# yassram/iterative-closest-point

Measured on AMD Instinct MI355X. Metric: ICP iterations/sec (synthetic 1048576-point pair, C4, exact NN), higher is better.
Workload: dtype f64 (30 exact fp64 grid searches (fp32 screen, candidates decided in fp64: the first from cell seeds, the seeded ones the fused grid iteration nn_grid_iter2_kernel, 75% of its queries kept their correspondence by the exclusion certificate without a walk); fp64 transform and reductions)

## Files before the change

### iterative-closest-point_amd/csrc/icp_grid.hip

```cpp
#include <hip/hip_runtime.h>

#include <algorithm>
#include <cmath>
#include <cstdlib>
#include <string>
#include <type_traits>

#include "icp_canon.h"
#include "icp_device.h"
#include "icp_gridbox.h"
#include "icp_kernels.h"

namespace icp {
namespace {

__device__ __forceinline__ double d64g(double px, double py, double pz, double mx, double my,
                                       double mz)
{
    const double dx = px - mx;
    const double dy = py - my;
    const double dz = pz - mz;
    return (dx * dx + dy * dy) + dz * dz;
}

// ... 951 lines not shown
                            const float rem = rc2 - dy * dy - dz * dz;
                            if (rem < 0.0f) {
                                x1 = x0 - 1;
                            } else {
                                const float xw = sqrtf(rem) * (1.0f + 0x1.0p-20f) + xroom;
                                x0 = max(x0, c0[0] + (int)floorf(fmaxf(tr[0] - xw, -1.0f)));
                                x1 = min(x1, c0[0] + (int)floorf(fminf(tr[0] + xw, xspan)));
                            }
#endif
                            if (x0 <= x1) {
                                a0 = gv.start[row + x0];
                                a1 = gv.start[row + x1 + 1];
                            }
                        }
                        k0[v] = a0;
                        pre[v + 1] = pre[v] + (a1 - a0);
                    }
                    if constexpr (kBal) {
                        int K[2 * KR], P[2 * KR + 1];
                        P[0] = 0;
#pragma unroll
                        for (int v = 0; v < KR; ++v) {
                            const int len = pre[v + 1] - pre[v];
                            const int ok0 = __builtin_amdgcn_update_dpp(0, k0[v], 0xB1, 0xf, 0xf, true);
                            const int ol = __builtin_amdgcn_update_dpp(0, len, 0xB1, 0xf, 0xf, true);
                            K[2 * v] = sub ? ok0 : k0[v];
                            K[2 * v + 1] = sub ? k0[v] : ok0;
                            P[2 * v + 1] = P[2 * v] + (sub ? ol : len);
                            P[2 * v + 2] = P[2 * v + 1] + (sub ? len : ol);
                        }
                        const int T = P[2 * KR];
                        for (int f0 = 0; f0 < T; f0 += G * KU) {
                            int kk[KU];
#pragma unroll
                            for (int v = 0; v < KU; ++v) {
                                const int f = f0 + sub + G * v;
                                int pp = K[0] + f;
#pragma unroll
                                for (int w = 1; w < 2 * KR; ++w)
                                    if (f >= P[w]) pp = K[w] + (f - P[w]);
                                kk[v] = f < T ? pp : -1;
                            }
                            float4 mm[KU];
#pragma unroll
                            for (int v = 0; v < KU; ++v) mm[v] = gv.pts32[kk[v] >= 0 ? kk[v] : 0];
#pragma unroll
                            for (int v = 0; v < KU; ++v)
                                if (kk[v] >= 0) test(mm[v], kk[v]);
                        }
                        continue;
                    }
                    const int tot = pre[KR];
                    for (int f0 = 0; f0 < tot; f0 += KU) {
                        int kk[KU];
#pragma unroll
                        for (int v = 0; v < KU; ++v) {
                            const int f = f0 + v;
                            int pp = k0[0] + f;
#pragma unroll
                            for (int w = 1; w < KR; ++w)
                                if (f >= pre[w]) pp = k0[w] + (f - pre[w]);
                            kk[v] = f < tot ? pp : -1;
                        }
                        float4 mm[KU];
#pragma unroll
                        for (int v = 0; v < KU; ++v) mm[v] = gv.pts32[kk[v] >= 0 ? kk[v] : 0];
#pragma unroll
                        for (int v = 0; v < KU; ++v)
                            if (kk[v] >= 0) test(mm[v], kk[v]);
                    }
                }
            }
            if (nc) flush();
        }
        lap(7);
#pragma unroll
        for (int o = 1; o < G; o <<= 1) {
            const double ob = __shfl_xor(best, o, 64);
            const int oi = __shfl_xor(bi, o, 64), ok2 = __shfl_xor(bk, o, 64), ows = __shfl_xor(wset, o, 64);
            const double ox = __shfl_xor(wx, o, 64), oy = __shfl_xor(wy, o, 64), oz = __shfl_xor(wz, o, 64);
            if (ob < best || (ob == best && (unsigned)oi < (unsigned)bi)) {
                best = ob;
                bi = oi;
                bk = ok2;
                wx = ox;
                wy = oy;
                wz = oz;
                wset = ows;
            } else if (ob == best && oi == bi) {
                bk = max(bk, ok2);
                if (!wset && ows) {
                    wx = ox;
                    wy = oy;
                    wz = oz;
                    wset = 1;
                }
            }
        }
        unsigned long long bigm = __ballot(active && !ok && sub == 0);
        nbig += __popcll(bigm);
        if (kIterDbg && dbg) dcnt[3] += __popcll(bigm);
        while (bigm) {
            const int bl = __ffsll((long long)bigm) - 1;
            bigm &= bigm - 1;
            const double bq[3] = {__shfl(q[0], bl, 64), __shfl(q[1], bl, 64), __shfl(q[2], bl, 64)};
            const double be = __shfl(e, bl, 64);
            const int bh = __shfl(h, bl, 64);
            double b2 = INFINITY;
            int bj = -1;
            int d0[3], d1[3];
            if (bh >= 0 && be == be && be < INFINITY && complete_box(bq, be, gv, budget, d0, d1)) {
                b2 = be;
                bj = bh;
                scan_box<64>(bq, d0, d1, gv, lane, b2, bj);
            } else {
                for (int k = lane; k < nm; k += 64) {
                    const double4 m = m4[k];
                    lex_min(b2, bj, d64g(bq[0], bq[1], bq[2], m.x, m.y, m.z), k);
                }
            }
            group_lex_min<64>(b2, bj);
            if (lane / G == bl / G) {
                best = b2;
                bi = bj < 0 ? 0 : bj;
                bk = -1;
                wset = 0;
            }
        }
        lap(8);
        if (active) {
            if (!(ok && bi == h)) {
                if (wset) {
                    y[0] = wx;
                    y[1] = wy;
                    y[2] = wz;
                } else {
                    const double4 w = m4[bi];
                    y[0] = w.x;
                    y[1] = w.y;
                    y[2] = w.z;
                }
            }
            if (sub == 0) {
                idx[t] = bi;
                yx[t] = y[0];
                yy[t] = y[1];
                yz[t] = y[2];
            }
        }
        const IterState *sh_ = fresh();
        const double cp[3] = {sh_->shift_p[0], sh_->shift_p[1], sh_->shift_p[2]};
        const double cy[3] = {sh_->shift_y[0], sh_->shift_y[1], sh_->shift_y[2]};
        const double d[6] = {active ? q[0] - cp[0] : 0.0, active ? q[1] - cp[1] : 0.0, active ? q[2] - cp[2] : 0.0,
                             active ? y[0] - cy[0] : 0.0, active ? y[1] - cy[1] : 0.0, active ? y[2] - cy[2] : 0.0};
        if constexpr (G == 2 && ICP_ITER_LDS_TREE) {
            double *const lf = s_leaf[wave];
#pragma unroll
            for (int k = 0; k < kCanonCols; ++k) {
                double leaf;
                if (k < 6) leaf = 0.0 + d[k];
                else if (k < 15) leaf = 0.0 + d[(k - 6) / 3] * d[3 + (k - 6) % 3];
                else if (k == 15) leaf = 0.0 + ((d[3] * d[3] + d[4] * d[4]) + d[5] * d[5]);
                else if (k == 16) leaf = 0.0 + ((d[0] * d[0] + d[1] * d[1]) + d[2] * d[2]);
                else leaf = active ? 0.0 + e : 0.0;
                if (!active) leaf = 0.0;
                if (sub == 0) lf[k * kLeafStride + u] = leaf;
            }
            __builtin_amdgcn_fence(__ATOMIC_RELEASE, "wavefront");
            __builtin_amdgcn_wave_barrier();
            __builtin_amdgcn_fence(__ATOMIC_ACQUIRE, "wavefront");
            if (lane < kCanonCols) {
                const double *col = lf + lane * kLeafStride;
                double part[4];
#pragma unroll
                for (int g8 = 0; g8 < 4; ++g8) {
                    double v[8];
#pragma unroll
                    for (int j = 0; j < 8; ++j) v[j] = col[8 * g8 + j];
                    part[g8] = ((v[0] + v[1]) + (v[2] + v[3])) + ((v[4] + v[5]) + (v[6] + v[7]));
                }
                acc = acc + ((part[0] + part[1]) + (part[2] + part[3]));
            }
            __builtin_amdgcn_fence(__ATOMIC_RELEASE, "wavefront");
            __builtin_amdgcn_wave_barrier();
            __builtin_amdgcn_fence(__ATOMIC_ACQUIRE, "wavefront");
        } else
#pragma unroll
        for (int k = 0; k < kCanonCols; ++k) {
            double leaf;
            if (k < 6) leaf = 0.0 + d[k];
            else if (k < 15) leaf = 0.0 + d[(k - 6) / 3] * d[3 + (k - 6) % 3];
            else if (k == 15) leaf = 0.0 + ((d[3] * d[3] + d[4] * d[4]) + d[5] * d[5]);
            else if (k == 16) leaf = 0.0 + ((d[0] * d[0] + d[1] * d[1]) + d[2] * d[2]);
            else leaf = active ? 0.0 + e : 0.0;
            if (!active) leaf = 0.0;
            if constexpr (G == 2) {
                const double v = lane_value(wave_tree_odd(leaf), 63);
                if (lane == k) acc = acc + v;
            } else {
                const double v = lane_value(wave_tree_quad(leaf), 63);
                if (lane == k) acc = v;
            }
        }
        lap(9);
    }
    if (kIterDbg && dbg)
        for (int o = 32; o >= 1; o >>= 1) dcnt[4] += __shfl_xor(dcnt[4], o, 64);
    if (kIterDbg && dbg && lane == 0)
        for (int f = 0; f < 12; ++f)
            if (dcnt[f]) atomicAdd(dbg + f, dcnt[f]);
    __shared__ double sh[NW][kCanonCols];
    if (lane < kCanonCols) sh[wave][lane] = acc;
    __syncthreads();
    if (threadIdx.x < kCanonCols) {
        const int k = threadIdx.x;
        double v[4];
#pragma unroll
        for (int j = 0; j < 4; ++j)
            v[j] = H == 1 ? sh[j][k] : 0.0 + (sh[H * j][k] + sh[H * j + H - 1][k]);
        rows[(size_t)k * R + wr] = (v[0] + v[1]) + (v[2] + v[3]);
    }
    __shared__ int s_cnt[2][NW];
    for (int o = 32; o >= 1; o >>= 1) far += __shfl_xor(far, o, 64);
    if (lane == 0) {
        s_cnt[0][wave] = far;
        s_cnt[1][wave] = nbig;
    }
    __syncthreads();
    if (threadIdx.x < 2) {
        int tot = 0;
        for (int w = 0; w < NW; ++w) tot += s_cnt[threadIdx.x][w];
        int *dst = threadIdx.x == 0 ? far_acc : big_count;
        if (tot && dst) atomicAdd(dst, tot);
    }
}

constexpr int kNoBound = (int)0xbf800000u;
constexpr int kIter2Slot = 8;
constexpr int kIter2Tile = kCanonCols * kLeafStride;
static_assert(32 * kIter2Slot + 32 / 2 <= kIter2Tile, "the hand-off slots and the walker list alias the tiles");

#ifndef ICP_ITER2_DBG
#define ICP_ITER2_DBG 0
#endif
#ifndef ICP_ITER2_F64
#define ICP_ITER2_F64 0
#endif
#ifndef ICP_ITER2_KU
#define ICP_ITER2_KU 4
#endif
#ifndef ICP_ITER2_KR
#define ICP_ITER2_KR 3
#endif
#ifndef ICP_ITER2_KCAND
#define ICP_ITER2_KCAND ICP_ITER_KCAND
#endif
#ifndef ICP_ITER2_WAVES
#define ICP_ITER2_WAVES 4
#endif
#ifndef ICP_ITER2_GFLOOR
#define ICP_ITER2_GFLOOR 1
#endif
#ifndef ICP_ITER2_NWG_DEFAULT
#define ICP_ITER2_NWG_DEFAULT 1
#endif
struct Iter2Args {
    int n;
    double *px, *py, *pz, *yx, *yy, *yz;
    int *idx;
    const IterState *st;
    float4 *p32;
    GridView gv;
    int box, budget, nm;
    const double4 *m4;
    double *rows;
    int *far_acc;
    double far_d2;
    int *big_count;
    int xform, xcd_l;
    CertArgs ca;
    unsigned long long *dbg;
};
static_assert(std::is_trivially_copyable<Iter2Args>::value, "passed by value in the kernel-argument segment");
#define ICP_CONST_AS __attribute__((address_space(4)))
__device__ __forceinline__ const Iter2Args &iter2_args()
{
    auto *p = (const ICP_CONST_AS Iter2Args *)__builtin_amdgcn_kernarg_segment_ptr();
    asm volatile("" : "+s"(p));
    return *(const Iter2Args *)p;
}
__device__ __forceinline__ const IterState &iter2_state(const IterState *st)
{
    auto *p = (const ICP_CONST_AS IterState *)st;
    asm volatile("" : "+s"(p));
    return *(const IterState *)p;
}

template <bool A32, class T> __device__ __forceinline__ T &at32(T *b, int i)
{
    if constexpr (A32) return *(T *)((char *)b + (unsigned)i * (unsigned)sizeof(T));
    else return b[i];
}

template <int KR, int KU, int CH, int NWG, bool A32>
__global__ __launch_bounds__(64 * NWG) __attribute__((amdgpu_waves_per_eu(ICP_ITER2_WAVES))) void nn_grid_iter2_kernel(
    Iter2Args args_)
{
    static_assert(CH == 1 || CH == 2, "one or two chunks a task");
    constexpr bool kDbg = ICP_ITER2_DBG != 0;
    unsigned long long dcnt[4] = {0, 0, 0, 0};
    static_assert(NWG == 4 || NWG == 1, "a row or a strand a workgroup");
    constexpr int NW = NWG, QL = 2 / CH;
    __shared__ double s_tile[NW][CH * kIter2Tile];
    const Iter2Args &T = iter2_args();
    const IterState *const st = T.st;
    const unsigned long long dbg_t0 = kDbg ? __builtin_amdgcn_s_memrealtime() : 0ull;
    const int *const ord = NWG == 1 ? T.ca.order : nullptr;
    auto *oaddr = ord ? (const ICP_CONST_AS int *)ord + blockIdx.x : (const ICP_CONST_AS int *)&st->done;
    auto *daddr = (const ICP_CONST_AS int *)&st->done;
    int s_ord, done;
    asm volatile("s_load_dword %0, %2, 0x0\n\ts_load_dword %1, %3, 0x0\n\ts_waitcnt lgkmcnt(0)"
                 : "=&s"(done), "=&s"(s_ord)
                 : "s"(daddr), "s"(oaddr)
                 : "memory");
    if (done) return;
    const int n = T.n, xcd_l = T.xcd_l, xform = T.xform;
    const int lane = threadIdx.x & 63, wave = threadIdx.x >> 6, u = lane / QL, sub = lane % QL;
    const int C = canon_chunks((size_t)n), S = canon_strands((size_t)n), R = canon_rows((size_t)n);
    const int s = NWG == 4 ? xcd_row((int)blockIdx.x, R, xcd_l) * 4 + wave
                : ord ? ((unsigned)s_ord < (unsigned)S ? s_ord : S)
                      : xcd_row((int)blockIdx.x, S, xcd_l > 0 ? 4 * xcd_l : xcd_l);
    const int wr = s >> 2;
    double *const tile = s_tile[wave];
    double *const slots = tile;
    int *const wl = (int *)(tile + 32 * CH * kIter2Slot);
    auto at = [](auto *b, int i) -> auto & { return at32<A32>(b, i); };
    const bool cert_on = T.ca.state != nullptr, cert_in = cert_on && T.ca.valid != 0, two = T.ca.two != 0;
    auto wave_sync = [] {
        __builtin_amdgcn_fence(__ATOMIC_RELEASE, "wavefront");
        __builtin_amdgcn_wave_barrier();
        __builtin_amdgcn_fence(__ATOMIC_ACQUIRE, "wavefront");
    };
    double acc = 0.0;
    int far = 0, nbig = 0, ncert = 0, nwalk = 0;
    auto slot_t = [&](int c, int uu) { return (c + (uu >> 5) * S) * kCanonChunk + (uu & 31); };
    for (int c = s; s < S && c < C; c += CH * S) {
        const int t = slot_t(c, u);
        const bool active = c + (u >> 5) * S < C && t < n;
        if (kDbg) dcnt[0] += 1;
        const Iter2Args &A = iter2_args();
        const Xform xf = iter2_state(st).xf;
        double *const px = A.px, *const py = A.py, *const pz = A.pz, *const yx = A.yx, *const yy = A.yy, *const yz = A.yz;
        int *const idx = A.idx;
        int4 *const cstate = A.ca.state;
        float4 *const p32 = A.p32;
        const double far_d2 = A.far_d2;
        double q[3] = {0.0, 0.0, 0.0}, y[3] = {0.0, 0.0, 0.0};
        int h = -1;
        int4 cs4 = make_int4(kNoBound, kNoBound, -1, -1);
        double mot = 0.0;
        if (active) {
            const double p0 = at(px, t), p1 = at(py, t), p2 = at(pz, t);
            y[0] = at(yx, t);
            y[1] = at(yy, t);
            y[2] = at(yz, t);
            h = at(idx, t);
            if (cert_in) cs4 = at(cstate, t);
            if (xform) {
                transform_point(xf, p0, p1, p2, q[0], q[1], q[2]);
                if (cert_in)
                    mot = (double)(__builtin_amdgcn_sqrtf(__double2float_ru(residual2(p0, p1, p2, q[0], q[1], q[2]))) *
                                   (1.0f + 0x1.0p-21f));
            } else {
                q[0] = p0;
                q[1] = p1;
                q[2] = p2;
            }
        }
        const double e = active ? residual2(y[0], y[1], y[2], q[0], q[1], q[2]) : 0.0;
        if (active && sub == 0 && xform) {
            at(px, t) = q[0];
            at(py, t) = q[1];
            at(pz, t) = q[2];
            if (p32)
                at(p32, t) = make_float4((float)(q[0] - xf.c[0]), (float)(q[1] - xf.c[1]), (float)(q[2] - xf.c[2]),
                                     0.0f);
        }
        if (active && sub == 0) {
            if (far_d2 >= 0.0) {
                if (xform) far += e > far_d2 ? 1 : 0;
            } else if (!(h >= 0 && e * (A.gv.inv_h * A.gv.inv_h) < 2.2)) {
                int b0[3], b1[3];
                far += h >= 0 && e == e && e < INFINITY && complete_box(q, e, A.gv, A.box, b0, b1) ? 0 : 1;
            }
        }
        double best = e;
        int bi = h;
        double w[3] = {y[0], y[1], y[2]};
        bool certd = false;
        const float R1 = __int_as_float(cs4.x), R3 = __int_as_float(cs4.y);
        if (cert_in && active && h >= 0 && (R1 > 0.0f || R3 > 0.0f)) {
            const double R1c = ((double)R1 - mot) - (double)R1 * 0x1.0p-48;
            const double R3c = ((double)R3 - mot) - (double)R3 * 0x1.0p-48;
            auto inside = [](double d2, double r) { return r > 0.0 && d2 * (1.0 + 0x1.0p-38) < r * r * (1.0 - 0x1.0p-50); };
            double R1n = R1c;
            int2 pn = make_int2(cs4.z, cs4.w);
            certd = inside(e, R1c);
            if (kDbg && !certd && two && cs4.w >= 0 && R3c > 0.0) dcnt[3] += 1;
            if (!certd && two && cs4.w >= 0 && R3c > 0.0) {
                const double4 r2 = at(A.gv.pts, cs4.w);
                const double d2 = d64g(q[0], q[1], q[2], r2.x, r2.y, r2.z);
                const int mi2 = (int)r2.w;
                const bool swap = d2 < e || (d2 == e && (unsigned)mi2 < (unsigned)h);
                const double db = swap ? d2 : e;
                if (inside(db, R3c)) {
                    certd = true;
                    const double lb = fmin(R3c, (double)__builtin_amdgcn_sqrtf(__double2float_rd(swap ? e : d2)) * (1.0 - 0x1.0p-21));
                    if (swap) {
                        best = d2;
                        bi = mi2;
                        w[0] = r2.x;
                        w[1] = r2.y;
                        w[2] = r2.z;
                        R1n = lb;
                        pn = make_int2(cs4.w, cs4.z);
                    } else {
                        R1n = fmax(R1c, lb);
                    }
                }
            }
            if (certd && sub == 0) {
                const int4 ns = make_int4(__float_as_int(R1n > 0.0 ? __double2float_rd(R1n) : -1.0f),
                                          __float_as_int(R3c > 0.0 ? __double2float_rd(R3c) : -1.0f), pn.x, pn.y);
                if (bi != h) {
                    at(cstate, t) = ns;
                    at(idx, t) = bi;
                    at(yx, t) = w[0];
                    at(yy, t) = w[1];
                    at(yz, t) = w[2];
                } else {
                    *(int2 *)&at(cstate, t) = make_int2(ns.x, ns.y);
                }
            }
        }
        double *const sl = slots + u * kIter2Slot;
        const bool walker = active && !certd;
        if (walker && sub == 0) {
            sl[0] = q[0];
            sl[1] = q[1];
            sl[2] = q[2];
            sl[3] = best;
            ((int *)(sl + 7))[0] = bi;
            ((int *)(sl + 7))[1] = h;
        }
        if (active && sub == 0) {
            sl[4] = w[0];
            sl[5] = w[1];
            sl[6] = w[2];
        }
        const unsigned long long wm = __ballot(walker && sub == 0);
        ncert += certd && sub == 0 ? 1 : 0;
        nwalk += walker && sub == 0 ? 1 : 0;
        const int nW = __popcll(wm);
        if (walker && sub == 0) wl[__popcll(wm & ((1ull << lane) - 1ull))] = u;
        wave_sync();
        if (kDbg) dcnt[1] += nW;
        for (int b0 = 0; b0 < nW; b0 += 32) {
            const Iter2Args &D = iter2_args();
            const GridView gv = D.gv;
            const int box = D.box;
            const double skin = D.ca.skin;
            if (kDbg) dcnt[2] += 1;
            const int nb = min(32, nW - b0);
            const int lg = nb > 16 ? 1 : nb > 8 ? 2 : nb > 4 ? 3 : nb > 2 ? 4 : nb > 1 ? 5 : 6;
            const int G = ICP_ITER2_GFLOOR ? 64 / nb : 1 << lg;
            const int ginv = (65536 + G - 1) / G;
            const int wi = (lane * ginv) >> 16, ws = lane - wi * G, gbase = wi * G;
            const bool wact = wi < nb;
            const int wu = wl[b0 + (wact ? wi : 0)];
            const double *const ws_sl = slots + wu * kIter2Slot;
            double wq[3], wb = INFINITY;
            int wbi = -1;
            wq[0] = ws_sl[0];
            wq[1] = ws_sl[1];
            wq[2] = ws_sl[2];
            if (wact) {
                wb = ws_sl[3];
                wbi = ((const int *)(ws_sl + 7))[0];
            }
            int c0[3] = {0, 0, 0}, c1[3] = {-1, -1, -1};
            double rw = 0.0, rb = 0.0, s0 = 0.0;
            bool ok = false;
            if (wact && wbi >= 0 && wb == wb && wb < INFINITY) {
                s0 = sqrt(wb);
                if (cert_on) {
                    rw = s0 + skin;
                    rb = rw * (1.0 + 0x1.0p-51);
                    ok = complete_box_r(wq, rb, gv, box, c0, c1);
                }
                if (!ok) {
                    rw = rb = s0;
                    ok = complete_box_r(wq, rb, gv, box, c0, c1);
                }
            }
            if (wact && ws == 0) slots[wu * kIter2Slot + 3] = rw;
            int bk = -1;
            float a1 = INFINITY, a2 = INFINITY;
            int k1 = -1;
            auto other = [&](float v, int k) {
                const bool lt = v < a1;
                a2 = __builtin_amdgcn_fmed3f(a1, v, a2);
                a1 = lt ? v : a1;
                k1 = lt ? k : k1;
            };
            auto eq_of = [&]() {
                const double o0 = wq[0] - gv.c32[0], o1 = wq[1] - gv.c32[1], o2 = wq[2] - gv.c32[2];
                return std::ldexp(fmax(fabs(o0), fmax(fabs(o1), fabs(o2))), -23) + gv.em32;
            };
            double eq = 0.0;
            if (ok) {
                const float f0 = (float)(wq[0] - gv.c32[0]), f1 = (float)(wq[1] - gv.c32[1]), f2 = (float)(wq[2] - gv.c32[2]);
                eq = eq_of();
                const float T = seeded_bound32_root(s0, eq);
                const int ny = c1[1] - c0[1] + 1, nrq = ny * (c1[2] - c0[2] + 1);
                constexpr int kCand = ICP_ITER2_KCAND;
                int cand[kCand], nc = 0;
                auto flush = [&]() {
                    double4 r[kCand];
#pragma unroll
                    for (int j = 0; j < kCand; ++j)
                        if (j < nc) r[j] = at(gv.pts, cand[j]);
#pragma unroll
                    for (int j = 0; j < kCand; ++j) {
                        if (j >= nc) break;
                        const int mi = (int)r[j].w;
                        const double d = d64g(wq[0], wq[1], wq[2], r[j].x, r[j].y, r[j].z);
                        if (d < wb || (d == wb && (unsigned)mi < (unsigned)wbi)) {
                            if (cert_on && bk >= 0) other(__double2float_rd(wb), bk);
                            wb = d;
                            wbi = mi;
                            bk = cand[j];
                        } else if (cert_on) {
                            other(__double2float_rd(d), cand[j]);
                        }
                    }
                    nc = 0;
                };
                auto test = [&](const float4 (&m)[KU], const int (&kk)[KU]) {
                    bool cnd[KU];
                    bool anyc = false;
#pragma unroll
                    for (int v = 0; v < KU; ++v) {
                        const float dx = f0 - m[v].x, dy = f1 - m[v].y, dz = f2 - m[v].z;
                        const float d32 = (dx * dx + dy * dy) + dz * dz;
                        const bool val = kk[v] >= 0, fr = d32 > T;
                        if (cert_on) other(val && fr ? d32 : INFINITY, kk[v]);
                        const bool self = val && !fr && __float_as_int(m[v].w) == wbi;
                        bk = self ? kk[v] : bk;
                        cnd[v] = val && !fr && !self;
                        anyc = anyc || cnd[v];
                    }
                    if (__ballot(anyc)) {
#pragma unroll
                        for (int v = 0; v < KU; ++v)
                            if (cnd[v]) {
                                cand[nc++] = kk[v];
                                if (nc == kCand) flush();
                            }
                    }
                };
                const float inv_ny = 1.0f / (float)ny;
                float tr[3];
#pragma unroll
                for (int a = 0; a < 3; ++a) tr[a] = (float)((wq[a] - gv.lo[a]) * gv.inv_h - (double)c0[a]);
                const float rcf = (float)(rb * gv.inv_h * (1.0 + 0x1.0p-18) +
                                          0x1.0p-20 * (1.0 + fabs((double)tr[0]) + fabs((double)tr[1]) + fabs((double)tr[2])));
                const float rc2 = rcf * rcf, xroom = 0x1.0p-20f * (1.0f + fabsf(tr[0]));
                const float xspan = (float)(c1[0] - c0[0] + 1);
                auto row_run = [&](int r, int &a0, int &a1r) {
                    a0 = 0;
                    a1r = 0;
                    if (r >= nrq) return;
                    const int rz = (int)(((float)r + 0.5f) * inv_ny), ry = r - rz * ny;
                    const int row = ((c0[2] + rz) * gv.g[1] + c0[1] + ry) * gv.g[0];
                    int x0 = c0[0], x1 = c1[0];
                    const float dy = fmaxf(0.0f, fmaxf((float)ry - tr[1], tr[1] - (float)(ry + 1)));
                    const float dz = fmaxf(0.0f, fmaxf((float)rz - tr[2], tr[2] - (float)(rz + 1)));
                    const float rem = rc2 - dy * dy - dz * dz;
                    if (rem < 0.0f) return;
                    const float xw = __builtin_amdgcn_sqrtf(rem) * (1.0f + 0x1.0p-20f) + xroom;
                    x0 = max(x0, c0[0] + (int)floorf(fmaxf(tr[0] - xw, -1.0f)));
                    x1 = min(x1, c0[0] + (int)floorf(fminf(tr[0] + xw, xspan)));
                    if (x0 <= x1) {
                        a0 = at(gv.start, row + x0);
                        a1r = at(gv.start, row + x1 + 1);
                    }
                };
                {
                    for (int r0 = ws; r0 < nrq; r0 += KR * G) {
                        int k0[KR], pre[KR + 1];
                        pre[0] = 0;
#pragma unroll
                        for (int v = 0; v < KR; ++v) {
                            int a0, a1r;
                            row_run(r0 + v * G, a0, a1r);
                            k0[v] = a0;
                            pre[v + 1] = pre[v] + (a1r - a0);
                        }
                        const int tot = pre[KR];
                        for (int f0 = 0; f0 < tot; f0 += KU) {
                            int kk[KU];
#pragma unroll
                            for (int v = 0; v < KU; ++v) {
                                const int f = f0 + v;
                                int pp = k0[0] + f;
#pragma unroll
                                for (int x = 1; x < KR; ++x)
                                    if (f >= pre[x]) pp = k0[x] + (f - pre[x]);
                                kk[v] = f < tot ? pp : -1;
                            }
                            if constexpr (ICP_ITER2_F64) {
                                double4 mm[KU];
#pragma unroll
                                for (int v = 0; v < KU; ++v) mm[v] = at(gv.pts, kk[v] >= 0 ? kk[v] : 0);
#pragma unroll
                                for (int v = 0; v < KU; ++v) {
                                    const double d = d64g(wq[0], wq[1], wq[2], mm[v].x, mm[v].y, mm[v].z);
                                    const int mi = (int)mm[v].w, kv = kk[v];
                                    const bool val = kv >= 0, self = val && mi == wbi;
                                    const bool win = val && !self && (d < wb || (d == wb && (unsigned)mi < (unsigned)wbi));
                                    if (cert_on) {
                                        const float ov = win ? (bk >= 0 ? (float)wb * 0x1.fffffcp-1f : INFINITY)
                                                             : (val && !self ? (float)d * 0x1.fffffcp-1f : INFINITY);
                                        other(ov, win ? bk : kv);
                                    }
                                    wb = win ? d : wb;
                                    wbi = win ? mi : wbi;
                                    bk = win || self ? kv : bk;
                                }
                            } else {
                                float4 mm[KU];
#pragma unroll
                                for (int v = 0; v < KU; ++v) mm[v] = at(gv.pts32, kk[v] >= 0 ? kk[v] : 0);
                                test(mm, kk);
                            }
                        }
                    }
                }
                if constexpr (!ICP_ITER2_F64)
                    if (nc) flush();
            }
            for (int o = 1; o < G; o <<= 1) {
                const int pw = ws ^ o;
                const bool pin = pw < G;
                const int pl = gbase + (pin ? pw : ws);
                const double ob = pin ? __shfl(wb, pl, 64) : INFINITY;
                const int oi = pin ? __shfl(wbi, pl, 64) : -1, ok2 = pin ? __shfl(bk, pl, 64) : -1;
                const bool theirs = ob < wb || (ob == wb && (unsigned)oi < (unsigned)wbi);
                if (cert_on) {
                    const float oa1 = pin ? __shfl(a1, pl, 64) : INFINITY, oa2 = pin ? __shfl(a2, pl, 64) : INFINITY;
                    const int ok1 = pin ? __shfl(k1, pl, 64) : -1;
                    if (a1 <= oa1) {
                        a2 = fminf(a2, oa1);
                    } else {
                        a2 = fminf(oa2, a1);
                        a1 = oa1;
                        k1 = ok1;
                    }
                    if (oi != wbi) {
                        const int lk = theirs ? bk : ok2;
                        if (lk >= 0) other((float)(theirs ? wb : ob) * 0x1.fffffcp-1f, lk);
                    }
                }
                if (theirs) {
                    wb = ob;
                    wbi = oi;
                    bk = ok2;
                } else if (ob == wb && oi == wbi) {
                    bk = max(bk, ok2);
                }
            }
            unsigned long long bigm = __ballot(wact && ws == 0 && !ok);
            nbig += __popcll(bigm);
            bool whole = false;
            while (bigm) {
                const int bl = __ffsll((long long)bigm) - 1;
                bigm &= bigm - 1;
                const Iter2Args &B = iter2_args();
                const double bq[3] = {__shfl(wq[0], bl, 64), __shfl(wq[1], bl, 64), __shfl(wq[2], bl, 64)};
                const double be = __shfl(wb, bl, 64);
                const int bh = __shfl(wbi, bl, 64);
                double b2 = INFINITY;
                int bj = -1;
                int d0[3], d1[3];
                if (bh >= 0 && be == be && be < INFINITY && complete_box(bq, be, B.gv, B.budget, d0, d1)) {
                    b2 = be;
                    bj = bh;
                    scan_box<64>(bq, d0, d1, B.gv, lane, b2, bj);
                } else {
                    for (int k = lane; k < B.nm; k += 64) {
                        const double4 m = B.m4[k];
                        lex_min(b2, bj, d64g(bq[0], bq[1], bq[2], m.x, m.y, m.z), k);
                    }
                }
                group_lex_min<64>(b2, bj);
                if (wi == ((bl * ginv) >> 16)) {
                    wb = b2;
                    wbi = bj < 0 ? 0 : bj;
                    whole = true;
                }
            }
            if (wact && ws == 0) {
                const Iter2Args &O = iter2_args();
                int *const o_idx = O.idx;
                double *const o_yx = O.yx, *const o_yy = O.yy, *const o_yz = O.yz;
                int4 *const o_state = O.ca.state;
                const double4 *const o_pts = O.gv.pts;
                double *const rs_sl = slots + wu * kIter2Slot;
                const int seed = ((const int *)(rs_sl + 7))[0], wh = ((const int *)(rs_sl + 7))[1];
                const int wt = slot_t(c, wu);
                if (wbi != seed) {
                    const double4 m = whole ? at(O.m4, wbi) : at(o_pts, bk);
                    rs_sl[4] = m.x;
                    rs_sl[5] = m.y;
                    rs_sl[6] = m.z;
                }
                if (wbi != wh) {
                    at(o_idx, wt) = wbi;
                    at(o_yx, wt) = rs_sl[4];
                    at(o_yy, wt) = rs_sl[5];
                    at(o_yz, wt) = rs_sl[6];
                }
                if (cert_on) {
                    int4 ns = make_int4(kNoBound, kNoBound, -1, -1);
                    if (ok && !whole && bk >= 0) {
                        const double u0 = rs_sl[3] * (1.0 - 0x1.0p-40);
                        const double ec = ICP_ITER2_F64 ? 0.0 : 1.7320508075688774 * eq * (1.0 + 0x1.0p-20);
                        auto lower = [&](float a) {
                            return a < INFINITY ? fmin(u0, (double)__builtin_amdgcn_sqrtf(a) * (1.0 - 0x1.0p-20) - ec) : u0;
                        };
                        const double r1 = lower(a1), r3 = two ? lower(a2) : -1.0;
                        ns = make_int4(__float_as_int(r1 > 0.0 ? __double2float_rd(r1) : -1.0f),
                                       __float_as_int(r3 > 0.0 ? __double2float_rd(r3) : -1.0f), bk, two ? k1 : -1);
                    }
                    at(o_state, wt) = ns;
                }
            }
            wave_sync();
        }
        if (active) {
            y[0] = sl[4];
            y[1] = sl[5];
            y[2] = sl[6];
        }
        wave_sync();
        const IterState &sg = iter2_state(st);
        const double cp[3] = {sg.shift_p[0], sg.shift_p[1], sg.shift_p[2]};
        const double cy[3] = {sg.shift_y[0], sg.shift_y[1], sg.shift_y[2]};
        const double d[6] = {active ? q[0] - cp[0] : 0.0, active ? q[1] - cp[1] : 0.0, active ? q[2] - cp[2] : 0.0,
                             active ? y[0] - cy[0] : 0.0, active ? y[1] - cy[1] : 0.0, active ? y[2] - cy[2] : 0.0};
        double *const lf = tile + (u >> 5) * kIter2Tile;
#pragma unroll
        for (int k = 0; k < kCanonCols; ++k) {
            double leaf;
            if (k < 6) leaf = 0.0 + d[k];
            else if (k < 15) leaf = 0.0 + d[(k - 6) / 3] * d[3 + (k - 6) % 3];
            else if (k == 15) leaf = 0.0 + ((d[3] * d[3] + d[4] * d[4]) + d[5] * d[5]);
            else if (k == 16) leaf = 0.0 + ((d[0] * d[0] + d[1] * d[1]) + d[2] * d[2]);
            else leaf = active ? 0.0 + e : 0.0;
            if (sub == 0) lf[k * kLeafStride + (u & 31)] = leaf;
        }
        wave_sync();
        double tv = 0.0;
        if ((lane & 31) < kCanonCols && (CH == 2 || lane < 32)) {
            const double *col = tile + (lane >> 5) * kIter2Tile + (lane & 31) * kLeafStride;
            double part[4];
#pragma unroll
            for (int g8 = 0; g8 < 4; ++g8) {
                double v[8];
#pragma unroll
                for (int j = 0; j < 8; ++j) v[j] = col[8 * g8 + j];
                part[g8] = ((v[0] + v[1]) + (v[2] + v[3])) + ((v[4] + v[5]) + (v[6] + v[7]));
            }
            tv = (part[0] + part[1]) + (part[2] + part[3]);
        }
        const double tb = CH == 2 ? __shfl(tv, (lane & 31) + 32, 64) : 0.0;
        if (lane < kCanonCols) {
            acc = acc + tv;
            if (CH == 2 && c + S < C) acc = acc + tb;
        }
        wave_sync();
    }
    const Iter2Args &E = iter2_args();
    unsigned long long *const dbg = E.dbg;
    if (kDbg && dbg && lane == 0 && NWG != 1)
        for (int f = 0; f < 4; ++f)
            if (dcnt[f]) atomicAdd(dbg + f, dcnt[f]);
    if constexpr (NWG == 4) {
        __shared__ double sh[NW][kCanonCols];
        if (lane < kCanonCols) sh[wave][lane] = acc;
        __syncthreads();
        if (threadIdx.x < kCanonCols) {
            const int k = threadIdx.x;
            E.rows[(size_t)k * R + wr] = (sh[0][k] + sh[1][k]) + (sh[2][k] + sh[3][k]);
        }
    } else if (s < S && lane < kCanonCols) {
        E.rows[(size_t)lane * S + s] = acc;
    }
    __shared__ int s_cnt[4][NW];
    for (int o = 32; o >= 1; o >>= 1) {
        far += __shfl_xor(far, o, 64);
        ncert += __shfl_xor(ncert, o, 64);
        nwalk += __shfl_xor(nwalk, o, 64);
    }
    if (lane == 0) {
        s_cnt[0][wave] = far;
        s_cnt[1][wave] = nbig;
        s_cnt[2][wave] = ncert;
        s_cnt[3][wave] = nwalk;
        if (NWG == 1 && E.ca.walk_last && s < S) E.ca.walk_last[s] = nwalk;
        if (kDbg && dbg && NWG == 1) {
            unsigned long long *const rec = dbg + 16 + 4 * (size_t)blockIdx.x;
            rec[0] = dbg_t0;
            rec[1] = __builtin_amdgcn_s_memrealtime();
            rec[2] = (unsigned long long)(unsigned)s << 32 | (unsigned long long)(blockIdx.x & 7) << 16 |
                     (unsigned long long)(nwalk & 0xffff);
            rec[3] = (dcnt[0] & 0xffffull) << 48 | (dcnt[2] & 0xffffull) << 32 | (dcnt[3] & 0xffffffffull);
        }
    }
    __syncthreads();
    if (threadIdx.x < 4) {
        int tot = 0;
        for (int w = 0; w < NW; ++w) tot += s_cnt[threadIdx.x][w];
        if (threadIdx.x < 2) {
            int *dst = threadIdx.x == 0 ? E.far_acc : E.big_count;
            if (tot && dst) atomicAdd(dst, tot);
        } else if (E.ca.counts && (NWG == 4 || s < S)) {
            E.ca.counts[2 * (NWG == 4 ? wr : s) + (threadIdx.x - 2)] += (unsigned long long)tot;
        }
    }
}

bool iter2_addr32(int n, int nm, const GridView &gv)
{
    const long long ncell = (long long)gv.g[0] * gv.g[1] * gv.g[2];
    return n <= (1 << 28) && nm <= (1 << 27) && ncell < (1ll << 30);
}

}

static int iter_xcd_l(int n)
{
    static const int xcd_env = [] {
        const char *e = getenv("ICP_ITER_XCD_L");
        return e ? atoi(e) : -2;
    }();
    return xcd_env != -2 ? xcd_env : (canon_chunks((size_t)n) >= 8192 ? 32 : -1);
}

int nn_grid_iter_strand_run(int n)
{
    const int xcd_l = iter_xcd_l(n);
    return xcd_l > 0 ? 4 * xcd_l : xcd_l;
}

bool launch_nn_grid_iter(int n, double *px, double *py, double *pz, double *yx, double *yy, double *yz, int *idx,
                         const IterState *st_dev, float4 *p32, const GridView &gv, int box, int budget, int nm,
                         const double4 *m4, double *rows, int *far_acc, double far_d2, int *big_count, hipStream_t st,
                         unsigned long long *dbg, int xform, const CertArgs &ca, int *strands)
{
    if (strands) *strands = 0;
    if (n <= 0) return false;
    static const bool stage = [] {
        const char *e = getenv("ICP_ITER_STAGE");
        return e && atoi(e) == 1;
    }();
    static const bool wide_on = [] {
        const char *e = getenv("ICP_ITER_WIDE");
        return e && atoi(e) == 1;
    }();
    const int R = canon_rows((size_t)n);
    const int xcd_l = iter_xcd_l(n);
    static const bool v2 = [] {
        const char *e = getenv("ICP_ITER_V2");
        return !(e && e[0] == '0');
    }();
    if (v2 && !stage && !(wide_on && n <= kIterWideMax) && (!dbg || ICP_ITER2_DBG)) {
        static const int ch = [] {
            const char *e = getenv("ICP_ITER2_CH");
            return e && atoi(e) == 1 ? 1 : 2;
        }();
        static const int nwg = [] {
            const char *e = getenv("ICP_ITER2_NWG");
            return e && atoi(e) == 4 ? 4 : ICP_ITER2_NWG_DEFAULT;
        }();
        const int S = canon_strands((size_t)n);
        if (strands) *strands = nwg == 1 ? S : 0;
        const Iter2Args ka{n,      px, py, pz,   yx,      yy,     yz,        idx,   st_dev, p32, gv, box,
                           budget, nm, m4, rows, far_acc, far_d2, big_count, xform, xcd_l,  ca,  dbg};
        static const bool a32_on = [] {
            const char *e = getenv("ICP_ITER2_A32");
            return !(e && e[0] == '0');
        }();
        const bool a32 = a32_on && iter2_addr32(n, nm, gv);
        auto launch = [&](auto chc, auto nwgc, auto a32c) {
            constexpr int kCh = decltype(chc)::value, kNwg = decltype(nwgc)::value;
            nn_grid_iter2_kernel<ICP_ITER2_KR, ICP_ITER2_KU, kCh, kNwg, decltype(a32c)::value>
                <<<kNwg == 1 ? S : R, 64 * kNwg, 0, st>>>(ka);
        };
        auto with_a32 = [&](auto chc, auto nwgc) {
            if (a32) launch(chc, nwgc, std::true_type{});
            else launch(chc, nwgc, std::false_type{});
        };
        using I1 = std::integral_constant<int, 1>;
        using I2 = std::integral_constant<int, 2>;
        using I4 = std::integral_constant<int, 4>;
        if (ch == 2 && nwg == 1) with_a32(I2{}, I1{});
        else if (ch == 2) with_a32(I2{}, I4{});
        else if (nwg == 1) with_a32(I1{}, I1{});
        else with_a32(I1{}, I4{});
        return ca.state != nullptr;
    }
    if (!stage && wide_on && n <= kIterWideMax)
        nn_grid_iter_kernel<false, 4><<<R, 2 * kBlock, 0, st>>>(n, px, py, pz, yx, yy, yz, idx, st_dev, p32, gv, box,
                                                                 budget, nm, m4, rows, far_acc, far_d2, big_count, dbg, xform, xcd_l);
    else if (stage)
        nn_grid_iter_kernel<true, 2><<<R, kBlock, 0, st>>>(n, px, py, pz, yx, yy, yz, idx, st_dev, p32, gv, box,
                                                            budget, nm, m4, rows, far_acc, far_d2, big_count, dbg, xform, xcd_l);
    else
        nn_grid_iter_kernel<false, 2><<<R, kBlock, 0, st>>>(n, px, py, pz, yx, yy, yz, idx, st_dev, p32, gv, box,
                                                             budget, nm, m4, rows, far_acc, far_d2, big_count, dbg, xform, xcd_l);
    return false;
}

namespace {
}

GridParams grid_params(const double *m_xyz, size_t nm)
{
    double lo[3] = {INFINITY, INFINITY, INFINITY}, hi[3] = {-INFINITY, -INFINITY, -INFINITY};
    for (size_t j = 0; j < nm; ++j)
        for (int a = 0; a < 3; ++a) {
            lo[a] = std::min(lo[a], m_xyz[3 * j + a]);
            hi[a] = std::max(hi[a], m_xyz[3 * j + a]);
        }
    return grid_params_box(lo, hi, nm);
}

GridParams grid_params_box(const double lo[3], const double hi[3], size_t nm)
{
    GridParams p{};
    double ext[3], emax = 0.0;
    for (int a = 0; a < 3; ++a) {
        ext[a] = hi[a] - lo[a];
        emax = std::max(emax, ext[a]);
        p.lo[a] = lo[a];
        p.c32[a] = lo[a] + 0.5 * ext[a];
    }
    p.em32 = std::isfinite(emax) ? std::ldexp(emax, -23) : INFINITY;
    if (!(emax > 0.0) || !std::isfinite(emax)) {
        p.g[0] = p.g[1] = p.g[2] = 1;
        p.inv_h = 1.0;
        return p;
    }
    static const double ppc = [] {
        const char *e = getenv("ICP_GRID_PPC");
        const double v = e ? atof(e) : 0.0;
        return v > 0.0 ? v : 2.0;
    }();
    double vol = 1.0;
    for (int a = 0; a < 3; ++a) vol *= std::max(ext[a], emax * 1e-3);
    double h = std::cbrt(vol * ppc / (double)std::max<size_t>(nm, 1));
    auto dims = [&](double hh, int g[3]) {
        long long tot = 1;
        for (int a = 0; a < 3; ++a) {
            g[a] = (int)std::min<double>(std::floor(ext[a] / hh) + 1.0, 1 << 12);
            tot *= g[a];
        }
        return tot;
    };
    while (dims(h, p.g) > kGridMaxCells) h *= 1.25;
    p.inv_h = 1.0 / h;
    return p;
}

static bool grid_flat_scan(int g)
{
    static const int forced = [] {
        const char *e = getenv("ICP_GRID_SCAN");
        if (!e) return -1;
        return std::string(e) == "rows" ? 0 : (std::string(e) == "flat" ? 1 : -1);
    }();
    return forced >= 0 ? forced == 1 : g >= 16;
}

long long grid_cells(const GridParams &p) { return (long long)p.g[0] * p.g[1] * p.g[2]; }

static int cell_bits(long long ncell)
{
    int bits = 1;
    while (bits < 32 && (1ll << bits) <= ncell) ++bits;
    return bits;
}

static size_t grid_keys_bytes(int nm) { return (4 * (size_t)nm * sizeof(int) + 255) & ~(size_t)255; }

size_t grid_build_scratch_bytes(int nm, long long ncell)
{
    size_t temp = 0;
    (void)sort_pairs_u32(nullptr, temp, nullptr, nullptr, nullptr, nullptr, nm, cell_bits(ncell), nullptr);
    return grid_keys_bytes(nm) + ((temp + 255) & ~(size_t)255);
}

int launch_grid_build(const double *mx, const double *my, const double *mz, const double4 *m4, int nm,
                      const GridParams &p, void *scratch, size_t bytes, int *start, double4 *pts, float4 *pts32,
                      hipStream_t st)
{
    const long long ncell = grid_cells(p);
    GridView gv{};
    for (int a = 0; a < 3; ++a) {
        gv.g[a] = p.g[a];
        gv.lo[a] = p.lo[a];
    }
    gv.inv_h = p.inv_h;
    unsigned *k0 = (unsigned *)scratch, *k1 = k0 + nm;
    int *v0 = (int *)(k1 + nm), *v1 = v0 + nm;
    size_t temp_bytes = bytes - grid_keys_bytes(nm);
    const int g = (nm + kBlock - 1) / kBlock;
    static const bool fused = [] {
        const char *e = getenv("ICP_GRID_FUSED");
        return !(e && atoi(e) == 0);
    }();
    if (fused) v0 = nullptr;
    grid_keys_kernel<<<g, kBlock, 0, st>>>(mx, my, mz, nm, gv, k0, v0);
    if (sort_pairs_u32((char *)scratch + grid_keys_bytes(nm), temp_bytes, k0, k1, v0, v1, nm, cell_bits(ncell), st) !=
        hipSuccess)
        return -1;
    if (!fused) grid_starts_kernel<<<(int)((ncell + kBlock) / kBlock), kBlock, 0, st>>>(k1, nm, (int)ncell, start);
    grid_gather_kernel<<<g, kBlock, 0, st>>>(m4, nm, v1, pts, pts32, p.c32[0], p.c32[1], p.c32[2],
                                             fused ? k1 : nullptr, (int)ncell, start);
    return 0;
}

void launch_nn_grid_search(int np, const double *px, const double *py, const double *pz, const GridView &gv,
                           int budget, int *idx, int *fb_count, int *fb_list, double *fb_T, hipStream_t st)
{
    static const int forced = [] {
        const char *e = getenv("ICP_GRID_GROUP");
        return e ? atoi(e) : 0;
    }();
    const int g = forced == 4 || forced == 16 ? forced : (np >= (1 << 16) ? 4 : 16);
    const int per_block = kBlock / g;
    const int blocks = std::max(1, std::min((np + per_block - 1) / per_block, 16384));
#define SEARCH(GG, F) nn_grid_search_kernel<GG, F><<<blocks, kBlock, 0, st>>>(np, px, py, pz, gv, budget, idx, fb_count, fb_list, fb_T)
    if (grid_flat_scan(g)) {
        if (g == 4) SEARCH(4, true);
        else SEARCH(16, true);
    } else {
        if (g == 4) SEARCH(4, false);
        else SEARCH(16, false);
    }
#undef SEARCH
}

void launch_nn_grid_cell_seed(int n, const double *px, const double *py, const double *pz, const GridView &gv, int nm,
                              int *idx, double *seedd, hipStream_t st, double *yx, double *yy, double *yz)
{
    if (n <= 0) return;
    nn_grid_cell_seed_kernel<<<(n + kBlock - 1) / kBlock, kBlock, 0, st>>>(n, px, py, pz, gv, nm, idx, seedd, yx, yy,
                                                                          yz);
}

void launch_nn_grid_seed(int np, const double *px, const double *py, const double *pz, const GridView &gv,
                         int nm, int *idx, hipStream_t st)
{
    constexpr int kG = 4, kMaxRing = 2;
    const int per_block = kBlock / kG;
    const int blocks = std::max(1, std::min((np + per_block - 1) / per_block, 16384));
    if (grid_flat_scan(kG)) nn_grid_seed_kernel<kG, true><<<blocks, kBlock, 0, st>>>(np, px, py, pz, gv, kMaxRing, nm, idx);
    else nn_grid_seed_kernel<kG, false><<<blocks, kBlock, 0, st>>>(np, px, py, pz, gv, kMaxRing, nm, idx);
}

void launch_nn_grid_resolve(const int *count_ptr, int max_items, const int *list, const int *hint,
                            const double *px, const double *py, const double *pz, const double4 *m4,
                            const GridView &gv, int budget, int *idx, int *fb_count, int *fb_list,
                            const double *T_in, double *T_out, hipStream_t st, const int *stop, int inline_nm,
                            int *kpos, const int *kd_of, int group, double *yx, double *yy, double *yz)
{
    static const int forced = [] {
        const char *e = getenv("ICP_GRID_RGROUP");
        return e ? atoi(e) : 0;
    }();
    const int g = forced == 4 || forced == 16 || forced == 64 ? forced
                  : group == 4 || group == 16 || group == 64 ? group
                                                             : (max_items >= 8192 && max_items < (1 << 18) ? 64 : 16);
    const int per_block = kBlock / g;
    static const int cap = [] {
        const char *e = getenv("ICP_GRID_RBLOCKS");
        return e && atoi(e) > 0 ? atoi(e) : 4096;
    }();
    const int blocks = std::max(1, std::min((max_items + per_block - 1) / per_block, cap));
#define RESOLVE(GG, F)                                                                                  \
    nn_grid_resolve_kernel<GG, F><<<blocks, kBlock, 0, st>>>(count_ptr, list, hint, px, py, pz, m4, gv, budget, idx, \
                                                             fb_count, fb_list, T_in, T_out, stop, inline_nm, 0, \
                                                             kpos, kd_of, 0, nullptr, nullptr, nullptr, nullptr, yx, yy, yz)
    if (grid_flat_scan(g)) {
        if (g == 4) RESOLVE(4, true);
        else if (g == 64) RESOLVE(64, true);
        else RESOLVE(16, true);
    } else {
        if (g == 4) RESOLVE(4, false);
        else if (g == 64) RESOLVE(64, false);
        else RESOLVE(16, false);
    }
#undef RESOLVE
}

void launch_nn_grid_resolve_all(int n, const double *px, const double *py, const double *pz, const double4 *m4,
                                const GridView &gv, int budget, int *idx, int *fb_count, int *fb_list, double *fb_T,
                                hipStream_t st, const int *stop, int inline_nm, bool xcd_remap, int *far_count,
                                int *far_list, int *far_hint, int *kpos, const int *kd_of, const double *seedd)
{
    static const int forced = [] {
        const char *e = getenv("ICP_GRID_GROUP");
        return e ? atoi(e) : 0;
    }();
    const int g = forced == 4 || forced == 16 ? forced : (n >= (1 << 16) ? 4 : 16);
    const int per_block = kBlock / g;
    int blocks = std::max(1, std::min((n + per_block - 1) / per_block, 16384));
    if (xcd_remap) blocks = (blocks + 7) / 8 * 8;
#define RESOLVE_ALL(GG, F)                                                                                       \
    nn_grid_resolve_kernel<GG, F><<<blocks, kBlock, 0, st>>>(nullptr, nullptr, nullptr, px, py, pz, m4, gv, budget, \
                                                             idx, fb_count, fb_list, nullptr, fb_T, stop, inline_nm, n, \
                                                             kpos, kd_of, xcd_remap ? 1 : 0, far_count, far_list, far_hint, \
                                                             seedd, nullptr, nullptr, nullptr)
    if (grid_flat_scan(g)) {
        if (g == 4) RESOLVE_ALL(4, true);
        else RESOLVE_ALL(16, true);
    } else {
        if (g == 4) RESOLVE_ALL(4, false);
        else RESOLVE_ALL(16, false);
    }
#undef RESOLVE_ALL
}

void launch_nn_grid_seeded(int n, const double *px, const double *py, const double *pz, const GridView &gv,
                           int budget, const double *seedd, const double4 *m4, int *idx, double *yx, double *yy,
                           double *yz, int *far_count, int *far_list, int *far_hint, const int *stop, bool xcd_remap,
                           hipStream_t st, long long nm_hint)
{
    struct Form {
        const char *name;
        int g;
    };
    static const Form forms[] = {{"2,2,2", 2}, {"4,2,2", 4}, {"4,2,4", 4}, {"2,2,4", 2},  {"f2,2,4", 2},
                                 {"f2,2,2", 2}, {"f4,2,4", 4}, {"f2,4,4", 2}, {"f4,2,2", 4}, {"4,1,2", 4},
                                 {"f4,1,2", 4}};
    int forced = -1;
    if (const char *e = getenv("ICP_GRID_SEEDED"))
        for (int i = 0; i < (int)(sizeof(forms) / sizeof(forms[0])); ++i)
            if (std::string(e) == forms[i].name) forced = i;
    const int form = forced >= 0 ? forced : (n >= (1 << 19) && nm_hint < 2 * (long long)n) ? 0 : 1;
    static const int xcd_env = [] {
        const char *e = getenv("ICP_SEEDED_XCD_L");
        return e ? atoi(e) : -2;
    }();
    const int xcd_l = xcd_env != -2 ? xcd_env : xcd_remap ? -1 : 32;
    const int f = form >= 4 && form != 9 && !gv.pts32 ? 0 : form;
    const int per_block = kBlock / forms[f].g;
    int blocks = std::max(1, std::min((n + per_block - 1) / per_block, 16384));
    if (xcd_remap) blocks = (blocks + 7) / 8 * 8;
    const char *te = getenv("ICP_GRID_TRIM");
    const int trim = te ? (std::string(te) == "1" ? 1 : 0) : (f == 0 ? 1 : 0);
#define SEEDED(K, ...)                                                                                       \
    K<__VA_ARGS__><<<blocks, kBlock, 0, st>>>(n, px, py, pz, gv, budget, seedd, m4, idx, yx, yy, yz, far_count, \
                                              far_list, far_hint, stop, xcd_l, trim)
    static const int seeded_tb = [] {
        const char *e = getenv("ICP_SEEDED_TB");
        return e ? atoi(e) : 0;
    }();
    if (f == 0 && (seeded_tb == 64 || (seeded_tb != 256 && !xcd_remap))) {
        int b64 = std::max(1, std::min((n + 64 / 2 - 1) / (64 / 2), 65536));
        if (xcd_remap) b64 = (b64 + 7) / 8 * 8;
        nn_grid_seeded_kernel<2, 2, 2, 1, 64><<<b64, 64, 0, st>>>(n, px, py, pz, gv, budget, seedd, m4, idx, yx, yy, yz,
                                                                  far_count, far_list, far_hint, stop, xcd_l, trim);
        return;
    }
    switch (f) {
    case 1: SEEDED(nn_grid_seeded_kernel, 4, 2, 2, 1); break;
    case 2: SEEDED(nn_grid_seeded_kernel, 4, 2, 4, 1); break;
    case 3: SEEDED(nn_grid_seeded_kernel, 2, 2, 4, 1); break;
    case 4: SEEDED(nn_grid_seeded32_kernel, 2, 2, 4); break;
    case 5: SEEDED(nn_grid_seeded32_kernel, 2, 2, 2); break;
    case 6: SEEDED(nn_grid_seeded32_kernel, 4, 2, 4); break;
    case 7: SEEDED(nn_grid_seeded32_kernel, 2, 4, 4); break;
    case 8: SEEDED(nn_grid_seeded32_kernel, 4, 2, 2); break;
    case 9: SEEDED(nn_grid_seeded_kernel, 4, 1, 2, 1); break;
    case 10: SEEDED(nn_grid_seeded32_kernel, 4, 1, 2); break;
    default: SEEDED(nn_grid_seeded_kernel, 2, 2, 2, 1); break;
    }
#undef SEEDED
}

namespace {
template <int G>
__global__ __launch_bounds__(kBlock) void nn_cpu_rule_window_kernel(
    int n, const double *__restrict__ px, const double *__restrict__ py, const double *__restrict__ pz,
    const double4 *__restrict__ m4, GridView gv, int budget, const int *__restrict__ idx, int *__restrict__ count,
    CpuRuleEntry *__restrict__ out, int max_entries, const int *__restrict__ stop)
{
    if (stop && *stop) return;
    const int sub = threadIdx.x & (G - 1);
    const int groups = gridDim.x * (kBlock / G);
    for (int j = (blockIdx.x * kBlock + threadIdx.x) / G; j < n; j += groups) {
        const double q[3] = {px[j], py[j], pz[j]};
// ... 73 lines not shown
```

Baseline: 10850.

## Stash walker slots early, carry winner coords, drop +0.0 in leaf sums

Adds a template variant in which the second certificate candidate's point is loaded before the point write-back and far-count side work, so that load latency overlaps other work. Walker slots are written during that side work, and the walk now carries the winning candidate's coordinates in registers, so the final correspondence write no longer re-reads the match point from global memory unless the walk went to the whole cloud. A second flag drops the 0.0+ additions when building the reduction leaves. Both are on by default through environment toggles, and they add an extra wave sync plus more register pressure.

```diff
diff --git a/iterative-closest-point_amd/csrc/icp_grid.hip b/iterative-closest-point_amd/csrc/icp_grid.hip
--- a/iterative-closest-point_amd/csrc/icp_grid.hip
+++ b/iterative-closest-point_amd/csrc/icp_grid.hip
@@ -1277,11 +1277,12 @@
     else return b[i];
 }
 
-template <int KR, int KU, int CH, int NWG, bool A32>
+template <int KR, int KU, int CH, int NWG, bool A32, int V>
 __global__ __launch_bounds__(64 * NWG) __attribute__((amdgpu_waves_per_eu(ICP_ITER2_WAVES))) void nn_grid_iter2_kernel(
     Iter2Args args_)
 {
     static_assert(CH == 1 || CH == 2, "one or two chunks a task");
+    constexpr bool kStash = (V & 1) != 0, kBare = (V & 2) != 0;
     constexpr bool kDbg = ICP_ITER2_DBG != 0;
     unsigned long long dcnt[4] = {0, 0, 0, 0};
     static_assert(NWG == 4 || NWG == 1, "a row or a strand a workgroup");
@@ -1353,37 +1354,53 @@
             }
         }
         const double e = active ? residual2(y[0], y[1], y[2], q[0], q[1], q[2]) : 0.0;
-        if (active && sub == 0 && xform) {
-            at(px, t) = q[0];
-            at(py, t) = q[1];
-            at(pz, t) = q[2];
-            if (p32)
-                at(p32, t) = make_float4((float)(q[0] - xf.c[0]), (float)(q[1] - xf.c[1]), (float)(q[2] - xf.c[2]),
-                                     0.0f);
-        }
-        if (active && sub == 0) {
-            if (far_d2 >= 0.0) {
-                if (xform) far += e > far_d2 ? 1 : 0;
-            } else if (!(h >= 0 && e * (A.gv.inv_h * A.gv.inv_h) < 2.2)) {
-                int b0[3], b1[3];
-                far += h >= 0 && e == e && e < INFINITY && complete_box(q, e, A.gv, A.box, b0, b1) ? 0 : 1;
-            }
-        }
+        double *const sl = slots + u * kIter2Slot;
+        auto side_work = [&](bool settled1) {
+            if (active && sub == 0 && xform) {
+                at(px, t) = q[0];
+                at(py, t) = q[1];
+                at(pz, t) = q[2];
+                if (p32)
+                    at(p32, t) = make_float4((float)(q[0] - xf.c[0]), (float)(q[1] - xf.c[1]), (float)(q[2] - xf.c[2]),
+                                         0.0f);
+            }
+            if (active && sub == 0) {
+                if (far_d2 >= 0.0) {
+                    if (xform) far += e > far_d2 ? 1 : 0;
+                } else if (!(h >= 0 && e * (A.gv.inv_h * A.gv.inv_h) < 2.2)) {
+                    int b0[3], b1[3];
+                    far += h >= 0 && e == e && e < INFINITY && complete_box(q, e, A.gv, A.box, b0, b1) ? 0 : 1;
+                }
+            }
+            if (kStash && active && !settled1 && sub == 0) {
+                sl[0] = q[0];
+                sl[1] = q[1];
+                sl[2] = q[2];
+                sl[3] = e;
+                ((int *)(sl + 7))[0] = h;
+                ((int *)(sl + 7))[1] = h;
+            }
+        };
+        if constexpr (!kStash) side_work(false);
         double best = e;
         int bi = h;
         double w[3] = {y[0], y[1], y[2]};
         bool certd = false;
         const float R1 = __int_as_float(cs4.x), R3 = __int_as_float(cs4.y);
-        if (cert_in && active && h >= 0 && (R1 > 0.0f || R3 > 0.0f)) {
-            const double R1c = ((double)R1 - mot) - (double)R1 * 0x1.0p-48;
-            const double R3c = ((double)R3 - mot) - (double)R3 * 0x1.0p-48;
-            auto inside = [](double d2, double r) { return r > 0.0 && d2 * (1.0 + 0x1.0p-38) < r * r * (1.0 - 0x1.0p-50); };
+        const bool bounded = cert_in && active && h >= 0 && (R1 > 0.0f || R3 > 0.0f);
+        const double R1c = ((double)R1 - mot) - (double)R1 * 0x1.0p-48;
+        const double R3c = ((double)R3 - mot) - (double)R3 * 0x1.0p-48;
+        auto inside = [](double d2, double r) { return r > 0.0 && d2 * (1.0 + 0x1.0p-38) < r * r * (1.0 - 0x1.0p-50); };
+        if (bounded) certd = inside(e, R1c);
+        const bool pair = bounded && !certd && two && cs4.w >= 0 && R3c > 0.0;
+        if (kDbg && pair) dcnt[3] += 1;
+        double4 r2 = make_double4(0.0, 0.0, 0.0, 0.0);
+        if (pair) r2 = at(A.gv.pts, cs4.w);
+        if constexpr (kStash) side_work(certd);
+        if (bounded) {
             double R1n = R1c;
             int2 pn = make_int2(cs4.z, cs4.w);
-            certd = inside(e, R1c);
-            if (kDbg && !certd && two && cs4.w >= 0 && R3c > 0.0) dcnt[3] += 1;
-            if (!certd && two && cs4.w >= 0 && R3c > 0.0) {
-                const double4 r2 = at(A.gv.pts, cs4.w);
+            if (pair) {
                 const double d2 = d64g(q[0], q[1], q[2], r2.x, r2.y, r2.z);
                 const int mi2 = (int)r2.w;
                 const bool swap = d2 < e || (d2 == e && (unsigned)mi2 < (unsigned)h);
@@ -1418,9 +1435,8 @@
                 }
             }
         }
-        double *const sl = slots + u * kIter2Slot;
         const bool walker = active && !certd;
-        if (walker && sub == 0) {
+        if (!kStash && walker && sub == 0) {
             sl[0] = q[0];
             sl[1] = q[1];
             sl[2] = q[2];
@@ -1480,6 +1496,7 @@
             }
             if (wact && ws == 0) slots[wu * kIter2Slot + 3] = rw;
             int bk = -1;
+            double wc[3] = {0.0, 0.0, 0.0};
             float a1 = INFINITY, a2 = INFINITY;
             int k1 = -1;
             auto other = [&](float v, int k) {
@@ -1515,6 +1532,11 @@
                             wb = d;
                             wbi = mi;
                             bk = cand[j];
+                            if constexpr (kStash) {
+                                wc[0] = r[j].x;
+                                wc[1] = r[j].y;
+                                wc[2] = r[j].z;
+                            }
                         } else if (cert_on) {
                             other(__double2float_rd(d), cand[j]);
                         }
@@ -1612,6 +1634,11 @@
                                     wb = win ? d : wb;
                                     wbi = win ? mi : wbi;
                                     bk = win || self ? kv : bk;
+                                    if constexpr (kStash) {
+                                        wc[0] = win ? mm[v].x : wc[0];
+                                        wc[1] = win ? mm[v].y : wc[1];
+                                        wc[2] = win ? mm[v].z : wc[2];
+                                    }
                                 }
                             } else {
                                 float4 mm[KU];
@@ -1625,6 +1652,7 @@
                 if constexpr (!ICP_ITER2_F64)
                     if (nc) flush();
             }
+            const int wbi0 = wbi;
             for (int o = 1; o < G; o <<= 1) {
                 const int pw = ws ^ o;
                 const bool pin = pw < G;
@@ -1685,6 +1713,16 @@
                     whole = true;
                 }
             }
+            if constexpr (kStash) {
+                const int fwbi = __shfl(wbi, gbase, 64);
+                if (wact && !whole && wbi0 == fwbi && fwbi != ((const int *)(ws_sl + 7))[0]) {
+                    double *const rs_sl = slots + wu * kIter2Slot;
+                    rs_sl[4] = wc[0];
+                    rs_sl[5] = wc[1];
+                    rs_sl[6] = wc[2];
+                }
+                wave_sync();
+            }
             if (wact && ws == 0) {
                 const Iter2Args &O = iter2_args();
                 int *const o_idx = O.idx;
@@ -1694,7 +1732,7 @@
                 double *const rs_sl = slots + wu * kIter2Slot;
                 const int seed = ((const int *)(rs_sl + 7))[0], wh = ((const int *)(rs_sl + 7))[1];
                 const int wt = slot_t(c, wu);
-                if (wbi != seed) {
+                if (kStash ? whole && wbi != seed : wbi != seed) {
                     const double4 m = whole ? at(O.m4, wbi) : at(o_pts, bk);
                     rs_sl[4] = m.x;
                     rs_sl[5] = m.y;
@@ -1738,7 +1776,13 @@
 #pragma unroll
         for (int k = 0; k < kCanonCols; ++k) {
             double leaf;
-            if (k < 6) leaf = 0.0 + d[k];
+            if constexpr (kBare) {
+                if (k < 6) leaf = d[k];
+                else if (k < 15) leaf = d[(k - 6) / 3] * d[3 + (k - 6) % 3];
+                else if (k == 15) leaf = (d[3] * d[3] + d[4] * d[4]) + d[5] * d[5];
+                else if (k == 16) leaf = (d[0] * d[0] + d[1] * d[1]) + d[2] * d[2];
+                else leaf = e;
+            } else if (k < 6) leaf = 0.0 + d[k];
             else if (k < 15) leaf = 0.0 + d[(k - 6) / 3] * d[3 + (k - 6) % 3];
             else if (k == 15) leaf = 0.0 + ((d[3] * d[3] + d[4] * d[4]) + d[5] * d[5]);
             else if (k == 16) leaf = 0.0 + ((d[0] * d[0] + d[1] * d[1]) + d[2] * d[2]);
@@ -1878,14 +1922,26 @@
             return !(e && e[0] == '0');
         }();
         const bool a32 = a32_on && iter2_addr32(n, nm, gv);
-        auto launch = [&](auto chc, auto nwgc, auto a32c) {
+        static const int form = [] {
+            const char *s = getenv("ICP_ITER2_STASH"), *b = getenv("ICP_ITER2_BARE");
+            return (s && s[0] == '0' ? 0 : 1) | (b && b[0] == '0' ? 0 : 2);
+        }();
+        auto launch = [&](auto chc, auto nwgc, auto a32c, auto vc) {
             constexpr int kCh = decltype(chc)::value, kNwg = decltype(nwgc)::value;
-            nn_grid_iter2_kernel<ICP_ITER2_KR, ICP_ITER2_KU, kCh, kNwg, decltype(a32c)::value>
+            nn_grid_iter2_kernel<ICP_ITER2_KR, ICP_ITER2_KU, kCh, kNwg, decltype(a32c)::value, decltype(vc)::value>
                 <<<kNwg == 1 ? S : R, 64 * kNwg, 0, st>>>(ka);
         };
+        auto with_form = [&](auto chc, auto nwgc, auto a32c) {
+            using I0 = std::integral_constant<int, 0>;
+            using I3 = std::integral_constant<int, 3>;
+            if (form == 3) launch(chc, nwgc, a32c, I3{});
+            else if (form == 2) launch(chc, nwgc, a32c, std::integral_constant<int, 2>{});
+            else if (form == 1) launch(chc, nwgc, a32c, std::integral_constant<int, 1>{});
+            else launch(chc, nwgc, a32c, I0{});
+        };
         auto with_a32 = [&](auto chc, auto nwgc) {
-            if (a32) launch(chc, nwgc, std::true_type{});
-            else launch(chc, nwgc, std::false_type{});
+            if (a32) with_form(chc, nwgc, std::true_type{});
+            else with_form(chc, nwgc, std::false_type{});
         };
         using I1 = std::integral_constant<int, 1>;
         using I2 = std::integral_constant<int, 2>;
```

After: 10900, median of 6. No clear change (+0.5%).
